# kkty/kmer-sets-compression

Hardware: AMD Instinct MI355X
Metric: Mk-mers/s processed in kmerset-multiple-compress; bytes/k-mer after SPSS (higher is better)
Workload: dtype u32

## Files before the change

kmer-sets-compression_amd/csrc/ksh_decode.hip:

```cpp
#include "ksh_internal.h"
#include "ksh_kmer.h"

#include <algorithm>
#include <cstdlib>
#include <string>
#include <vector>

namespace ksh {

constexpr int kDecThreads = 1024;
constexpr int kMaxLdsBuckets = 16384;
constexpr int kSortLdsBytes = 63488;
constexpr int kMaxSubBits = 11;
constexpr int kSortThreads = 1024;

__global__ __launch_bounds__(256) void k_str_bases(const uint32_t* __restrict__ lens, int64_t n,
                                                    int k, int64_t* __restrict__ bases) {
  const int64_t i = int64_t(blockIdx.x) * blockDim.x + threadIdx.x;
  if (i < n) bases[i] = int64_t(lens[i]) + k;
}

__global__ __launch_bounds__(256) void k_mark_ends(const int64_t* __restrict__ str_start,
                                                    int64_t n_strings,
                                                    unsigned long long* __restrict__ end_bits) {
// ... 46 lines not shown
    for (int j = 0; j < 32; j++) {
      const int64_t p = p0 + j;
      const bool valid = (p + k <= n_bases) && (((eb >> j) & no_end_mask) == 0);
      if (valid) {
        const uint64_t cn = (canonical_flag && rc < fw) ? rc : fw;
        const uint32_t bucket = uint32_t(cn >> key_bits);
        if (kScatter) {
          const uint32_t rel = atomicAdd(&lds_hist[bucket], 1u);
          keys[offsets[bucket] + rel] = KeyT(cn & key_mask);
        } else {
          atomicAdd(&lds_hist[bucket], 1u);
        }
      }
      const int q = j + k;
      const uint64_t nb = q < 32 ? (w0 >> (62 - 2 * q)) & 3 : (w1 >> (62 - 2 * (q - 32))) & 3;
      fw = ((fw << 2) & mask) | nb;
      rc = (rc >> 2) | ((3 - nb) << (2 * (k - 1)));
    }
  }
  if (!kScatter) {
    __syncthreads();
    for (int b = threadIdx.x; b < n_buckets; b += kDecThreads) my_row[b] = lds_hist[b];
  }
}

constexpr int kDecSgBits = 7;
constexpr int kDecL1Threads = 1024;
template <typename KeyT>
struct DecL1 {
  static constexpr int kPer = sizeof(KeyT) == 8 ? 4 : 8;
  static constexpr int kTile = kDecL1Threads * kPer;
};
constexpr int kDecL2Threads = 256;
constexpr int kDecL2Per = 8;
constexpr int kDecL2Tile = kDecL2Threads * kDecL2Per;

template <typename KeyT>
__global__ __launch_bounds__(kDecL1Threads) void k_decode_l1(
    const uint64_t* __restrict__ words, int64_t n_words, int64_t n_bases,
    const unsigned long long* __restrict__ end_bits, int64_t n_end_words, int k, int key_bits, int n_bucket_bits,
    int canonical_flag, int64_t words_per_group, const uint32_t* __restrict__ hist_matrix,
    const int64_t* __restrict__ offsets, KeyT* __restrict__ tmp_keys, uint16_t* __restrict__ tmp_b) {
  constexpr int kSg = 1 << kDecSgBits;
  constexpr int kDecL1Per = DecL1<KeyT>::kPer, kDecL1Tile = DecL1<KeyT>::kTile;
  constexpr int kParts = 32 / kDecL1Per;
  __shared__ KeyT s_key[kDecL1Tile];
  __shared__ uint16_t s_bkt[kDecL1Tile];
  __shared__ uint32_t s_cur[kSg], s_cnt[kSg], s_lbase[kSg + 1];
  const int tid = threadIdx.x;
  const int nb = 1 << n_bucket_bits, lo_bits = n_bucket_bits - kDecSgBits;
  const uint32_t* my_row = hist_matrix + int64_t(blockIdx.x) * nb;
  if (tid < kSg) {
    uint32_t at = uint32_t(offsets[int64_t(tid) << lo_bits]);
    for (int bi = 0; bi < (1 << lo_bits); bi++) at += my_row[(tid << lo_bits) + bi];
    s_cur[tid] = at;
    s_cnt[tid] = 0;
  }
  const int64_t w_begin = int64_t(blockIdx.x) * words_per_group;
  const int64_t w_end = min(w_begin + words_per_group, n_words);
  const uint64_t mask = kmer_mask(k);
  const uint64_t key_mask = (uint64_t(1) << key_bits) - 1;
  const uint64_t no_end_mask = (uint64_t(1) << (k - 1)) - 1;
  __syncthreads();
  for (int64_t w0i = w_begin; w0i < w_end; w0i += kDecL1Tile / 32) {
    const int64_t w = w0i + tid / kParts;
    const int j0 = (tid % kParts) * kDecL1Per;
    KeyT key[kDecL1Per];
    uint32_t bkt[kDecL1Per], rank[kDecL1Per];
// ... 36 lines not shown
      for (int d = 1; d < 64; d <<= 1) {
        const uint32_t o = __shfl_up(inc, d, 64);
        if (tid >= d) inc += o;
      }
      s_lbase[2 * tid] = inc - c0 - c1;
      s_lbase[2 * tid + 1] = inc - c1;
      if (tid == 63) s_lbase[kSg] = inc;
    }
    __syncthreads();
#pragma unroll
    for (int j = 0; j < kDecL1Per; j++) {
      if (bkt[j] == 0xFFFFFFFFu) continue;
      const uint32_t pos = s_lbase[bkt[j] >> lo_bits] + rank[j];
      s_key[pos] = key[j];
      s_bkt[pos] = uint16_t(bkt[j]);
    }
    __syncthreads();
    const int tile_n = int(s_lbase[kSg]);
    for (int i = tid; i < tile_n; i += kDecL1Threads) {
      const uint32_t sg = uint32_t(s_bkt[i]) >> lo_bits;
      const uint32_t dst = s_cur[sg] + (uint32_t(i) - s_lbase[sg]);
      tmp_keys[dst] = s_key[i];
      tmp_b[dst] = s_bkt[i];
    }
    __syncthreads();
    if (tid < kSg) {
      s_cur[tid] += s_cnt[tid];
      s_cnt[tid] = 0;
    }
    __syncthreads();
  }
}

template <typename KeyT>
__global__ __launch_bounds__(kDecL2Threads) void k_decode_l2(int64_t n, int n_bucket_bits,
                                                             const int64_t* __restrict__ offsets,
                                                             const KeyT* __restrict__ tmp_keys,
                                                             const uint16_t* __restrict__ tmp_b,
                                                             uint32_t* __restrict__ cursor, KeyT* __restrict__ keys) {
  constexpr int kBins = 2 * kDecL2Threads;
  __shared__ KeyT s_key[kDecL2Tile];
  __shared__ uint16_t s_bin[kDecL2Tile];
  __shared__ uint32_t s_cnt[kBins], s_lbase[kBins], s_gbase[kBins];
  __shared__ uint32_t s_wave[kDecL2Threads / 64];
  __shared__ uint32_t s_first;
  const int tid = threadIdx.x;
  const int lo_bits = n_bucket_bits - kDecSgBits;
  const int64_t p0 = int64_t(blockIdx.x) * kDecL2Tile;
  const int tile_n = int(min<int64_t>(kDecL2Tile, n - p0));
  s_cnt[2 * tid] = 0;
  s_cnt[2 * tid + 1] = 0;
  if (tid == 0) s_first = (uint32_t(tmp_b[p0]) >> lo_bits) << lo_bits;
  __syncthreads();
  const uint32_t base_b = s_first;
  const uint32_t n_bins = min<uint32_t>(uint32_t(kBins), (2u << lo_bits));
  KeyT mine[kDecL2Per];
  uint32_t bin[kDecL2Per], rank[kDecL2Per];
#pragma unroll
  for (int j = 0; j < kDecL2Per; j++) {
    const int i = tid + j * kDecL2Threads;
    bin[j] = 0xFFFFFFFFu;
    if (i >= tile_n) continue;
    mine[j] = tmp_keys[p0 + i];
    const uint32_t b = tmp_b[p0 + i];
    if (b - base_b < n_bins) {
      bin[j] = b - base_b;
      rank[j] = atomicAdd(&s_cnt[bin[j]], 1u);
    } else {
      keys[uint32_t(offsets[b]) + atomicAdd(&cursor[b], 1u)] = mine[j];
    }
  }
  __syncthreads();
  {
    const uint32_t c0 = s_cnt[2 * tid], c1 = s_cnt[2 * tid + 1];
    uint32_t inc = c0 + c1;
    const int lane = tid & 63, wv = tid >> 6;
#pragma unroll
    for (int d = 1; d < 64; d <<= 1) {
      const uint32_t o = __shfl_up(inc, d, 64);
      if (lane >= d) inc += o;
    }
    if (lane == 63) s_wave[wv] = inc;
    __syncthreads();
    uint32_t before = inc - (c0 + c1);
    for (int w = 0; w < wv; w++) before += s_wave[w];
    s_lbase[2 * tid] = before;
    s_lbase[2 * tid + 1] = before + c0;
    s_gbase[2 * tid] = c0 ? uint32_t(offsets[base_b + 2 * tid]) + atomicAdd(&cursor[base_b + 2 * tid], c0) : 0u;
    s_gbase[2 * tid + 1] = c1 ? uint32_t(offsets[base_b + 2 * tid + 1]) + atomicAdd(&cursor[base_b + 2 * tid + 1], c1) : 0u;
  }
  __syncthreads();
#pragma unroll
  for (int j = 0; j < kDecL2Per; j++) {
    if (bin[j] == 0xFFFFFFFFu) continue;
    const uint32_t pos = s_lbase[bin[j]] + rank[j];
    s_key[pos] = mine[j];
    s_bin[pos] = uint16_t(bin[j]);
  }
  __syncthreads();
  const uint32_t staged = s_lbase[kBins - 1] + s_cnt[kBins - 1];
  for (uint32_t i = tid; i < staged; i += kDecL2Threads) {
    const uint32_t b = s_bin[i];
    keys[s_gbase[b] + (i - s_lbase[b])] = s_key[i];
  }
}

constexpr int kColTeams = 16;
__global__ __launch_bounds__(64 * kColTeams) void k_hist_columns(uint32_t* __restrict__ hist_matrix,
                                                                  int64_t n_groups, int n_buckets,
                                                                  int64_t* __restrict__ totals,
                                                                  unsigned long long* __restrict__ max_total) {
  __shared__ uint32_t team_total[kColTeams][64];
  const int lane = threadIdx.x & 63, team = threadIdx.x >> 6;
  const int b = blockIdx.x * 64 + lane;
  const int64_t per_team = (n_groups + kColTeams - 1) / kColTeams;
  const int64_t g0 = min(int64_t(team) * per_team, n_groups), g1 = min(g0 + per_team, n_groups);
  uint32_t run = 0;
  if (b < n_buckets)
    for (int64_t g = g0; g < g1; g++) run += hist_matrix[g * n_buckets + b];
  team_total[team][lane] = run;
  __syncthreads();
  if (b >= n_buckets) return;
  uint32_t before = 0, all = 0;
#pragma unroll
  for (int t2 = 0; t2 < kColTeams; t2++) {
    const uint32_t v = team_total[t2][lane];
// ... 1 lines not shown
    all += v;
  }
  run = before;
  for (int64_t g = g0; g < g1; g++) {
    uint32_t* cell = hist_matrix + g * n_buckets + b;
    const uint32_t c = *cell;
    *cell = run;
    run += c;
  }
  if (team == 0) {
    totals[b] = all;
    unsigned long long m = all;
    if (int(blockIdx.x + 1) * 64 <= n_buckets) {
#pragma unroll
      for (int d = 32; d >= 1; d >>= 1) {
        const unsigned long long o = __shfl_xor(m, d, 64);
        m = o > m ? o : m;
      }
      if (lane == 0 && max_total) atomicMax(max_total, m);
    } else if (max_total) {
      atomicMax(max_total, m);
    }
  }
}

struct SortLds {
  uint32_t sub_cnt[(1 << kMaxSubBits) + 1];
  int wave_cnt[kSortThreads / 64];
  int wave_below[kSortThreads / 64];
  int overflow;
  int kept;
};

template <typename KeyT>
__device__ void block_sort_into_lds(const KeyT* __restrict__ src, int cnt, int eff_bits,
                                    KeyT* __restrict__ lds, SortLds* __restrict__ sh) {
  int bits = 0;
  while ((4 << bits) < cnt && bits < kMaxSubBits) bits++;
  if (bits > eff_bits) bits = eff_bits;
  const int n_sub = 1 << bits;
  const int shift = eff_bits - bits;
  for (int i = threadIdx.x; i <= n_sub; i += kSortThreads) sh->sub_cnt[i] = 0;
  if (threadIdx.x == 0) sh->overflow = 0;
  constexpr int kSortRegs = 8;
  const bool in_regs = cnt <= kSortRegs * kSortThreads;
  KeyT held[kSortRegs];
  if (in_regs) {
#pragma unroll
    for (int u = 0; u < kSortRegs; u++) {
      const int i = int(threadIdx.x) + u * kSortThreads;
      if (i < cnt) held[u] = src[i];
    }
  }
  __syncthreads();
  if (in_regs) {
#pragma unroll
    for (int u = 0; u < kSortRegs; u++)
      if (int(threadIdx.x) + u * kSortThreads < cnt)
        atomicAdd(&sh->sub_cnt[uint32_t(uint64_t(held[u]) >> shift) & uint32_t(n_sub - 1)], 1u);
  } else {
    for (int i = threadIdx.x; i < cnt; i += kSortThreads)
      atomicAdd(&sh->sub_cnt[uint32_t(uint64_t(src[i]) >> shift) & uint32_t(n_sub - 1)], 1u);
  }
  __syncthreads();
  {
    const int per = (n_sub + kSortThreads - 1) / kSortThreads;
    const int c0 = min(int(threadIdx.x) * per, n_sub), c1 = min(c0 + per, n_sub);
// ... 4 lines not shown
#pragma unroll
    for (int d = 1; d < 64; d <<= 1) {
      const int o = __shfl_up(inc, d, 64);
      if (lane >= d) inc += o;
    }
    if (lane == 63) sh->wave_cnt[wave] = inc;
    __syncthreads();
    int run = inc - mine;
    for (int w = 0; w < wave; w++) run += sh->wave_cnt[w];
    for (int i = c0; i < c1; i++) {
      const int c = int(sh->sub_cnt[i]);
      sh->sub_cnt[i] = uint32_t(run);
      run += c;
    }
  }
  __syncthreads();
  if (in_regs) {
#pragma unroll
    for (int u = 0; u < kSortRegs; u++)
      if (int(threadIdx.x) + u * kSortThreads < cnt) {
        const uint32_t pos = atomicAdd(&sh->sub_cnt[uint32_t(uint64_t(held[u]) >> shift) & uint32_t(n_sub - 1)], 1u);
        lds[pos] = held[u];
      }
  } else {
    for (int i = threadIdx.x; i < cnt; i += kSortThreads) {
      const KeyT key = src[i];
      const uint32_t pos = atomicAdd(&sh->sub_cnt[uint32_t(uint64_t(key) >> shift) & uint32_t(n_sub - 1)], 1u);
      lds[pos] = key;
    }
  }
  __syncthreads();
  for (int b2 = threadIdx.x; b2 < n_sub; b2 += kSortThreads) {
    const int s0 = b2 ? int(sh->sub_cnt[b2 - 1]) : 0, s1 = int(sh->sub_cnt[b2]);
    if (s1 - s0 > 64) {
      sh->overflow = 1;
    } else {
      for (int i = s0 + 1; i < s1; i++) {
        const KeyT x = lds[i];
        int j = i - 1;
        while (j >= s0 && lds[j] > x) {
          lds[j + 1] = lds[j];
          j--;
        }
        lds[j + 1] = x;
      }
    }
  }
  __syncthreads();
  if (sh->overflow == 0) return;
  int padded = 1;
  while (padded < cnt) padded <<= 1;
  const int half = padded >> 1;
  for (int size = 2; size <= padded; size <<= 1) {
    const int hs = size >> 1;
    for (int p = threadIdx.x; p < half; p += kSortThreads) {
      const int block = p / hs, o = p - block * hs;
      const int i = block * size + o, j = block * size + size - 1 - o;
      if (j < cnt) {
        const KeyT x = lds[i], y = lds[j];
        if (x > y) {
          lds[i] = y;
          lds[j] = x;
        }
      }
    }
    __syncthreads();
    for (int stride = size >> 2; stride > 0; stride >>= 1) {
      for (int p = threadIdx.x; p < half; p += kSortThreads) {
// ... 39 lines not shown
#pragma unroll
  for (int d = 32; d >= 1; d >>= 1) inc_below += __shfl_xor(inc_below, d, 64);
  __syncthreads();
  if (lane == 63) sh->wave_cnt[wave] = inc;
  if (lane == 0) sh->wave_below[wave] = inc_below;
  __syncthreads();
  int at = inc - mine;
  for (int w = 0; w < wave; w++) at += sh->wave_cnt[w];
  int total = 0;
#pragma unroll
  for (int w = 0; w < kSortThreads / 64; w++) total += sh->wave_cnt[w];
  if (threadIdx.x == 0 && below)
    for (int w = 0; w < kSortThreads / 64; w++) *below += sh->wave_below[w];
  if (total == cnt) {
    for (int i = threadIdx.x; i < cnt; i += kSortThreads) dst[i] = lds[i];
    __syncthreads();
    return total;
  }
  for (int i = c0; i < c1; i++) {
    if (i == 0 || lds[i] != lds[i - 1]) {
      bool keep = true;
      if (cutoff > 1) {
        int run = 1;
        while (run < cutoff && i + run < cnt && lds[i + run] == lds[i]) run++;
        keep = run >= cutoff;
      }
      if (keep) dst[at++] = lds[i];
    }
  }
  __syncthreads();
  return total;
}

template <typename KeyT>
__global__ __launch_bounds__(kSortThreads, 8) void k_bucket_sort(const int64_t* __restrict__ offsets,
                                                      KeyT* __restrict__ keys,
                                                      KeyT* __restrict__ scratch,
                                                      int64_t* __restrict__ uniq, int key_bits,
                                                      int cutoff, int64_t* __restrict__ below) {
  extern __shared__ unsigned char lds_raw[];
  __shared__ SortLds sh;
  __shared__ uint32_t part_end[(1 << kMaxSubBits) + 1];
  KeyT* lds = reinterpret_cast<KeyT*>(lds_raw);
  constexpr int kCap = kSortLdsBytes / int(sizeof(KeyT));
  const int64_t b = blockIdx.x;
  const int64_t lo = offsets[b], hi = offsets[b + 1];
  const int64_t cnt64 = hi - lo;
  if (cnt64 == 0) {
    if (threadIdx.x == 0) {
      uniq[b] = 0;
      if (below) below[b] = 0;
    }
    return;
  }
  KeyT* g = keys + lo;
  int64_t n_below = 0;
  if (cnt64 <= kCap) {
    block_sort_into_lds(g, int(cnt64), key_bits, lds, &sh);
    const int kept = block_unique_write(lds, int(cnt64), g, &sh, cutoff, &n_below);
    if (threadIdx.x == 0) {
      uniq[b] = kept;
      if (below) below[b] = n_below;
    }
    return;
  }
  KeyT* tmp = scratch + lo;
  int bits = 1;
  while ((cnt64 >> bits) > kCap / 4 && bits < kMaxSubBits) bits++;
  if (bits > key_bits) bits = key_bits;
  const int n_part = 1 << bits;
  const int shift = key_bits - bits;
  for (int i = threadIdx.x; i <= n_part; i += kSortThreads) part_end[i] = 0;
  __syncthreads();
  for (int64_t i = threadIdx.x; i < cnt64; i += kSortThreads)
    atomicAdd(&part_end[uint32_t(uint64_t(g[i]) >> shift) & uint32_t(n_part - 1)], 1u);
  __syncthreads();
  if (threadIdx.x == 0) {
    uint32_t run = 0;
    for (int i = 0; i < n_part; i++) {
      const uint32_t c = part_end[i];
      part_end[i] = run;
      run += c;
    }
  }
  __syncthreads();
  for (int64_t i = threadIdx.x; i < cnt64; i += kSortThreads) {
    const KeyT key = g[i];
    const uint32_t pos = atomicAdd(&part_end[uint32_t(uint64_t(key) >> shift) & uint32_t(n_part - 1)], 1u);
    tmp[pos] = key;
  }
  __syncthreads();
  int64_t out = 0;
  for (int p = 0; p < n_part; p++) {
    const int64_t s0 = p ? int64_t(part_end[p - 1]) : 0, s1 = int64_t(part_end[p]);
    const int64_t pc = s1 - s0;
    if (pc == 0) continue;
    if (pc <= kCap) {
      block_sort_into_lds(tmp + s0, int(pc), shift, lds, &sh);
      out += block_unique_write(lds, int(pc), g + out, &sh, cutoff, &n_below);
    } else {
      KeyT* buf = tmp + s0;
      int64_t padded = 1;
      while (padded < pc) padded <<= 1;
      const int64_t half = padded >> 1;
      for (int64_t size = 2; size <= padded; size <<= 1) {
        const int64_t hs = size >> 1;
        for (int64_t q = threadIdx.x; q < half; q += kSortThreads) {
          const int64_t block = q / hs, o = q - block * hs;
          const int64_t i = block * size + o, j = block * size + size - 1 - o;
          if (j < pc) {
            const KeyT x = buf[i], y = buf[j];
            if (x > y) {
              buf[i] = y;
              buf[j] = x;
            }
          }
        }
        __syncthreads();
        for (int64_t stride = size >> 2; stride > 0; stride >>= 1) {
          for (int64_t q = threadIdx.x; q < half; q += kSortThreads) {
            const int64_t i = 2 * stride * (q / stride) + (q % stride), j = i + stride;
            if (j < pc) {
              const KeyT x = buf[i], y = buf[j];
              if (x > y) {
                buf[i] = y;
                buf[j] = x;
              }
            }
          }
          __syncthreads();
        }
// ... 180 lines not shown
  ctx->dec_words = n_words;
  ctx->dec_groups = groups;
  ctx->dec_src = s->d_words;
  return KSH_OK;
}

template <typename KeyT>
int scatter_sort(ksh_ctx* ctx, const ksh_spss_view* s, const DecodeState& st, int k, int nbits_w, int kbw,
                 int canonical_flag, const int64_t* offsets, KeyT* keys, int cutoff, bool want_below,
                 int64_t** new_off, int64_t** below) {
  const int64_t nb = int64_t(1) << nbits_w;
  int64_t n_words, n_end_words, groups, wpg;
  decode_geometry(s, &n_words, &n_end_words, &groups, &wpg);
  static const bool direct = [] {
    const char* e = getenv("KSH_DECODE_SCATTER");
    return e && std::string(e) == "direct";
  }();
  static const int64_t two_level_min = [] {
    const char* e = getenv("KSH_DECODE_L2_MIN");
    return e ? std::max<int64_t>(1024, atoll(e)) : int64_t(1) << 20;
  }();
  if (!direct && ctx->dec_kmers >= two_level_min && nbits_w > kDecSgBits && nbits_w <= 15 &&
      ctx->dec_kmers < int64_t(0xFFFFFFF0)) {
    void* tmp = nullptr;
    const size_t tk = (size_t(ctx->dec_kmers) * sizeof(KeyT) + 255) & ~size_t(255);
    KSH_TRY(pool_alloc(ctx, tk + size_t(ctx->dec_kmers) * 2 + size_t(nb) * 4 + 256, &tmp));
    KeyT* tmp_keys = static_cast<KeyT*>(tmp);
    uint16_t* tmp_b = reinterpret_cast<uint16_t*>(static_cast<char*>(tmp) + tk);
    uint32_t* cursor = reinterpret_cast<uint32_t*>(static_cast<char*>(tmp) + tk + ((size_t(ctx->dec_kmers) * 2 + 255) & ~size_t(255)));
    KSH_HIP(hipMemsetAsync(cursor, 0, size_t(nb) * 4, ctx->stream));
    hipLaunchKernelGGL((k_decode_l1<KeyT>), dim3(unsigned(groups)), dim3(kDecL1Threads), 0, ctx->stream, s->d_words,
                       n_words, s->n_bases, st.end_bits, n_end_words, k, kbw, nbits_w,
                       canonical_flag, wpg, st.hist, offsets, tmp_keys, tmp_b);
    hipLaunchKernelGGL((k_decode_l2<KeyT>), dim3(unsigned((ctx->dec_kmers + kDecL2Tile - 1) / kDecL2Tile)),
                       dim3(kDecL2Threads), 0, ctx->stream, ctx->dec_kmers, nbits_w, offsets, tmp_keys, tmp_b,
                       cursor, keys);
    pool_free(ctx, tmp);
  } else {
    hipLaunchKernelGGL((k_decode<KeyT, true>), dim3(unsigned(groups)), dim3(kDecThreads),
                       size_t(nb) * 4, ctx->stream, s->d_words, n_words, s->n_bases, st.end_bits,
                       n_end_words, k, kbw, int(nb), canonical_flag, wpg, st.hist, offsets,
                       keys);
  }
  KeyT* scratch = nullptr;
  {
    const int64_t max_bucket = ctx->dec_max_bucket;
    if (max_bucket > int64_t(kSortLdsBytes / sizeof(KeyT))) {
      void* ptr = nullptr;
      KSH_TRY(pool_alloc(ctx, size_t(ctx->dec_kmers) * sizeof(KeyT), &ptr));
      scratch = static_cast<KeyT*>(ptr);
    }
  }
  arena_reset(ctx);
  KSH_TRY(arena_reserve(ctx, 2 * a256(size_t(nb + 1) * 8) + (1u << 16)));
  *new_off = static_cast<int64_t*>(arena_alloc(ctx, size_t(nb + 1) * 8));
  *below = static_cast<int64_t*>(arena_alloc(ctx, size_t(nb + 1) * 8));
  if (!*new_off || !*below) return fail(KSH_INTERNAL, "scratch arena too small");
  {
    const uint32_t bit = 8u << (sizeof(KeyT) == 2 ? 0 : sizeof(KeyT) == 4 ? 1 : 2);
    if (!(ctx->lds_opt_in & bit)) {
      KSH_HIP(hipFuncSetAttribute(reinterpret_cast<const void*>(k_bucket_sort<KeyT>),
                                  hipFuncAttributeMaxDynamicSharedMemorySize, kSortLdsBytes));
      ctx->lds_opt_in |= bit;
    }
  }
  hipLaunchKernelGGL((k_bucket_sort<KeyT>), dim3(unsigned(nb)), dim3(kSortThreads), kSortLdsBytes, ctx->stream,
                     offsets, keys, scratch, st.totals, kbw, cutoff, want_below ? *below : nullptr);
  if (scratch) pool_free(ctx, scratch);
  KSH_HIP(hipGetLastError());
  return KSH_OK;
}

template <typename KeyT, typename CT>
int decode_write_wide(ksh_ctx* ctx, const ksh_geom* g, const ksh_spss_view* s, int canonical_flag,
                      int64_t* d_offsets, void* d_keys, int64_t* n_keys, int cutoff, int64_t* n_below) {
  const int64_t nb = n_buckets(g), nbc = int64_t(1) << kCoarseBits;
  const int sub_bits = g->n_bucket_bits - kCoarseBits, cbits = 2 * g->k - kCoarseBits;
  int64_t n_words, n_end_words, groups, wpg;
  decode_geometry(s, &n_words, &n_end_words, &groups, &wpg);
  DecodeState st;
  decode_carve(ctx, groups, nbc, n_end_words, s->n_strings, &st);
  KeyT* keys = static_cast<KeyT*>(d_keys);
  constexpr bool in_place = sizeof(CT) == sizeof(KeyT);
  CT* comp = reinterpret_cast<CT*>(d_keys);
  if (!in_place) {
    void* ptr = nullptr;
    KSH_TRY(pool_alloc(ctx, size_t(ctx->dec_kmers) * sizeof(CT), &ptr));
    comp = static_cast<CT*>(ptr);
  }
  int64_t *new_off = nullptr, *below = nullptr;
  KSH_TRY(scatter_sort<CT>(ctx, s, st, g->k, kCoarseBits, cbits, canonical_flag, st.coarse, comp, cutoff,
                           n_below != nullptr, &new_off, &below));
  KSH_TRY(scan_exclusive_i64(ctx, st.totals, new_off, nbc, new_off + nbc));
  if (n_below) KSH_TRY(scan_exclusive_i64(ctx, below, below, nbc, below + nbc));
  hipLaunchKernelGGL((k_fine_offsets<CT>), dim3(unsigned(nb / 256 + 1)), dim3(256), 0, ctx->stream, st.coarse,
                     new_off, comp, sub_bits, key_bits(g), nb, d_offsets);
  KSH_HIP(hipMemcpyAsync(ctx->h_pinned, new_off + nbc, 8, hipMemcpyDeviceToHost, ctx->stream));
  if (n_below)
    KSH_HIP(hipMemcpyAsync(ctx->h_pinned + 1, below + nbc, 8, hipMemcpyDeviceToHost, ctx->stream));
  KSH_HIP(hipStreamSynchronize(ctx->stream));
// ... 139 lines not shown
```

kmer-sets-compression_amd/csrc/ksh_encode.hip:

```cpp
#include "ksh_internal.h"
#include "ksh_dsu.h"
#include "ksh_kmer.h"

#include <algorithm>
#include <cstddef>
#include <cstdlib>
#include <string>

namespace ksh {

#ifndef KSH_RULER_SHIFT
#define KSH_RULER_SHIFT 5
#endif
constexpr int kRulerShift = KSH_RULER_SHIFT;
constexpr uint32_t kRulerEvery = 1u << kRulerShift;

constexpr uint32_t kNone = 0xFFFFFFFFu;
constexpr uint32_t kMulti = 0xFFFFFFFEu;

#ifndef KSH_JUMP_HOPS
#define KSH_JUMP_HOPS 4
#endif
constexpr int kJumpHops = KSH_JUMP_HOPS;

// ... 204 lines not shown
                                                      RcRecord<KeyT>* __restrict__ rec) {
  extern __shared__ uint32_t lds_hist[];
  const int nb = 1 << nbits;
  const uint32_t* my_row = hist_matrix + int64_t(blockIdx.x) * nb;
  for (int b = threadIdx.x; b < nb; b += blockDim.x) lds_hist[b] = uint32_t(goff[b]) + my_row[b];
  const int64_t t_begin = int64_t(blockIdx.x) * per_row;
  const int64_t t_end = min(t_begin + per_row, set.n);
  __syncthreads();
  if (t_begin >= t_end) return;
  const int64_t b_first = set.bucket_of(t_begin), b_last = set.bucket_of(t_end - 1);
  const int k = set.k, low_bits = 2 * set.k - 2 - nbits;
  const uint64_t low_mask = (uint64_t(1) << low_bits) - 1;
  for (int64_t t = t_begin + threadIdx.x; t < t_end; t += blockDim.x) {
    const uint64_t key = uint64_t(set.keys[t]);
    const uint32_t grp = uint32_t(revcomp(key, k) >> low_bits) & uint32_t(nb - 1);
    if (int(grp >> (nbits - round_bits)) != round) continue;
    int64_t lo = b_first, hi = b_last;
    while (lo < hi) {
      const int64_t mid = (lo + hi + 1) >> 1;
      if (set.off[mid] <= t) lo = mid; else hi = mid - 1;
    }
    const uint64_t rx = revcomp((uint64_t(lo) << set.key_bits) | key, k);
    const uint32_t dst = atomicAdd(&lds_hist[grp], 1u);
    RcRecord<KeyT> r;
    r.key = KeyT(((rx >> (2 * k - 2)) << low_bits) | (rx & low_mask));
    r.t = uint32_t(t);
    rec[dst] = r;
  }
}

constexpr int kSgBits = 7;
constexpr int kL1Threads = 1024;
constexpr int kL2Threads = 256;
constexpr int kL2Per = 8;
constexpr int kL2Tile = kL2Threads * kL2Per;

template <typename KeyT, int kPer>
__global__ __launch_bounds__(kL1Threads) void k_rc_scatter_l1(DevSet<KeyT> set, int nbits, int64_t per_row,
                                                               const uint32_t* __restrict__ hist_matrix,
                                                               const int64_t* __restrict__ goff,
                                                               RcRecord<KeyT>* __restrict__ tmp_rec,
                                                               uint16_t* __restrict__ tmp_g) {
  constexpr int kTile = kL1Threads * kPer;
  constexpr int kSg = 1 << kSgBits;
  __shared__ RcRecord<KeyT> s_rec[kTile];
  __shared__ uint16_t s_g[kTile];
  __shared__ uint32_t s_cur[kSg], s_cnt[kSg], s_lbase[kSg + 1];
  constexpr int kOffCap = 1024;
  __shared__ int64_t s_off[kOffCap];
  const int tid = threadIdx.x;
  const int nb = 1 << nbits, lo_bits = nbits - kSgBits;
  const uint32_t* my_row = hist_matrix + int64_t(blockIdx.x) * nb;
  if (tid < kSg) {
    uint32_t at = uint32_t(goff[int64_t(tid) << lo_bits]);
    for (int gi = 0; gi < (1 << lo_bits); gi++) at += my_row[(tid << lo_bits) + gi];
    s_cur[tid] = at;
    s_cnt[tid] = 0;
  }
  const int64_t t_begin = int64_t(blockIdx.x) * per_row;
  const int64_t t_end = min(t_begin + per_row, set.n);
  __syncthreads();
  if (t_begin >= t_end) return;
  const int64_t b_first = set.bucket_of(t_begin), b_last = set.bucket_of(t_end - 1);
  const int k = set.k, low_bits = 2 * set.k - 2 - nbits;
  const uint64_t low_mask = (uint64_t(1) << low_bits) - 1;
  const int n_span = int(min<int64_t>(b_last - b_first + 1, kOffCap + 1));
  const bool off_staged = n_span <= kOffCap;
  if (off_staged)
// ... 36 lines not shown
      uint32_t inc = c0 + c1;
#pragma unroll
      for (int d = 1; d < 64; d <<= 1) {
        const uint32_t o = __shfl_up(inc, d, 64);
        if (tid >= d) inc += o;
      }
      s_lbase[2 * tid] = inc - c0 - c1;
      s_lbase[2 * tid + 1] = inc - c1;
    }
    __syncthreads();
#pragma unroll
    for (int j = 0; j < kPer; j++) {
      if (grp[j] == 0xFFFFFFFFu) continue;
      const uint32_t pos = s_lbase[grp[j] >> lo_bits] + rank[j];
      s_rec[pos] = mine[j];
      s_g[pos] = uint16_t(grp[j]);
    }
    __syncthreads();
    for (int i = tid; i < tile_n; i += kL1Threads) {
      const uint32_t sg = uint32_t(s_g[i]) >> lo_bits;
      const uint32_t dst = s_cur[sg] + (uint32_t(i) - s_lbase[sg]);
      tmp_rec[dst] = s_rec[i];
      tmp_g[dst] = s_g[i];
    }
    __syncthreads();
    if (tid < kSg) {
      s_cur[tid] += s_cnt[tid];
      s_cnt[tid] = 0;
    }
    __syncthreads();
  }
}

template <typename KeyT>
__global__ __launch_bounds__(kL2Threads) void k_rc_scatter_l2(int64_t n, int nbits, const int64_t* __restrict__ goff,
                                                               const RcRecord<KeyT>* __restrict__ tmp_rec,
                                                               const uint16_t* __restrict__ tmp_g,
                                                               uint32_t* __restrict__ cursor,
                                                               RcRecord<KeyT>* __restrict__ rec) {
  constexpr int kBins = 512;
  __shared__ RcRecord<KeyT> s_rec[kL2Tile];
  __shared__ uint16_t s_bin[kL2Tile];
  __shared__ uint32_t s_cnt[kBins], s_lbase[kBins], s_gbase[kBins];
  __shared__ uint32_t s_first;
  const int tid = threadIdx.x;
  const int lo_bits = nbits - kSgBits;
  const int64_t p0 = int64_t(blockIdx.x) * kL2Tile;
  const int tile_n = int(min<int64_t>(kL2Tile, n - p0));
  for (int b = tid; b < kBins; b += kL2Threads) s_cnt[b] = 0;
  if (tid == 0) s_first = (uint32_t(tmp_g[p0]) >> lo_bits) << lo_bits;
  __syncthreads();
  const uint32_t base_g = s_first;
  const uint32_t n_bins = min<uint32_t>(uint32_t(kBins), (2u << lo_bits));
  RcRecord<KeyT> mine[kL2Per];
  uint32_t bin[kL2Per], rank[kL2Per];
#pragma unroll
  for (int j = 0; j < kL2Per; j++) {
    const int i = tid + j * kL2Threads;
    bin[j] = 0xFFFFFFFFu;
    if (i >= tile_n) continue;
    mine[j] = tmp_rec[p0 + i];
    const uint32_t g = tmp_g[p0 + i];
    if (g - base_g < n_bins) {
      bin[j] = g - base_g;
      rank[j] = atomicAdd(&s_cnt[bin[j]], 1u);
    } else {
      rec[uint32_t(goff[g]) + atomicAdd(&cursor[g], 1u)] = mine[j];
    }
  }
  __syncthreads();
  {
    static_assert(kBins == 2 * kL2Threads, "two bins per thread");
    __shared__ uint32_t s_wave[kL2Threads / 64];
    const uint32_t c0 = s_cnt[2 * tid], c1 = s_cnt[2 * tid + 1];
    uint32_t inc = c0 + c1;
    const int lane = tid & 63, wv = tid >> 6;
#pragma unroll
    for (int d = 1; d < 64; d <<= 1) {
      const uint32_t o = __shfl_up(inc, d, 64);
      if (lane >= d) inc += o;
    }
    if (lane == 63) s_wave[wv] = inc;
    __syncthreads();
    uint32_t before = inc - (c0 + c1);
    for (int w = 0; w < wv; w++) before += s_wave[w];
    s_lbase[2 * tid] = before;
    s_lbase[2 * tid + 1] = before + c0;
    s_gbase[2 * tid] = c0 ? uint32_t(goff[base_g + 2 * tid]) + atomicAdd(&cursor[base_g + 2 * tid], c0) : 0u;
    s_gbase[2 * tid + 1] = c1 ? uint32_t(goff[base_g + 2 * tid + 1]) + atomicAdd(&cursor[base_g + 2 * tid + 1], c1) : 0u;
  }
  __syncthreads();
#pragma unroll
  for (int j = 0; j < kL2Per; j++) {
    if (bin[j] == 0xFFFFFFFFu) continue;
    const uint32_t pos = s_lbase[bin[j]] + rank[j];
    s_rec[pos] = mine[j];
    s_bin[pos] = uint16_t(bin[j]);
  }
  __syncthreads();
  uint32_t staged = 0;
  for (int b = 0; b < kBins; b++) staged += s_cnt[b];
  for (uint32_t i = tid; i < staged; i += kL2Threads) {
    const uint32_t b = s_bin[i];
    rec[s_gbase[b] + (i - s_lbase[b])] = s_rec[i];
  }
}

template <typename KeyT>
__device__ int64_t lower_bound_kmer(const DevSet<KeyT>& set, uint64_t value) {
  const int64_t b = int64_t(value >> set.key_bits);
  if (b >= set.n_buckets) return set.n;
  const KeyT key = KeyT(value & set.key_mask());
  int64_t lo, hi;
  set.probe_range(b, key, &lo, &hi);
  while (lo < hi) {
    const int64_t mid = (lo + hi) >> 1;
    if (set.keys[mid] < key) lo = mid + 1; else hi = mid;
  }
  return lo;
}

__device__ __forceinline__ void mark_hit(uint32_t* slot, uint32_t v) {
  if (atomicCAS(slot, kNone, v) != kNone) *reinterpret_cast<volatile uint32_t*>(slot) = kMulti;
}

constexpr int kRcSegs = 16;

template <typename KeyT>
__global__ __launch_bounds__(256) void k_rc_bounds(DevSet<KeyT> set, int nbits, int64_t* __restrict__ pb,
                                                    int64_t* __restrict__ pb0) {
  const int64_t i = int64_t(blockIdx.x) * blockDim.x + threadIdx.x;
  const int64_t n_pb = int64_t(2 * kRcSegs) << nbits;
  if (i < n_pb) {
    const uint64_t grp = uint64_t(i) >> 5, seg = (uint64_t(i) >> 1) & 15, which = uint64_t(i) & 1;
// ... 2706 lines not shown
          KSH_HIP(hipFuncSetAttribute(reinterpret_cast<const void*>(k_adj_rc<KeyT, 64>),
                                      hipFuncAttributeMaxDynamicSharedMemorySize, bytes));
          KSH_HIP(hipFuncSetAttribute(reinterpret_cast<const void*>(k_adj_rc1<KeyT, 1024>),
                                      hipFuncAttributeMaxDynamicSharedMemorySize, kRc1LdsBytes));
          KSH_HIP(hipFuncSetAttribute(reinterpret_cast<const void*>(k_adj_rc1<KeyT, 512>),
                                      hipFuncAttributeMaxDynamicSharedMemorySize, kRc1LdsBytes));
          KSH_HIP(hipFuncSetAttribute(reinterpret_cast<const void*>(k_adj_rc1<KeyT, 256>),
                                      hipFuncAttributeMaxDynamicSharedMemorySize, kRc1LdsBytes));
          KSH_HIP(hipFuncSetAttribute(reinterpret_cast<const void*>(k_adj_rc1<KeyT, 64>),
                                      hipFuncAttributeMaxDynamicSharedMemorySize, kRc1LdsBytes));
          KSH_HIP(hipFuncSetAttribute(reinterpret_cast<const void*>(k_rc_hist<KeyT>),
                                      hipFuncAttributeMaxDynamicSharedMemorySize, int(size_t(4) << 15)));
          ctx->lds_opt_in |= bit;
        }
      }
      KSH_BOUND(hist_lds <= (size_t(4) << 15) && ng <= 65536);
      hipLaunchKernelGGL((k_rc_hist<KeyT>), dim3(unsigned(rows)), dim3(1024), hist_lds, st,
                         static_cast<const KeyT*>(sv->d_keys), n, g->k, key_bits(g), gbits, per_row, hist);
      hipLaunchKernelGGL(k_rc_columns, dim3(unsigned((ng + 63) / 64)), dim3(64 * kColTeams), 0, st, hist, rows, int(ng),
                         totals);
      KSH_TRY(scan_exclusive_i64(ctx, totals, goff, ng, goff + ng));
      p->routes |= KSH_ROUTE_PROBE_STAGED | (two_level ? KSH_ROUTE_SCATTER_TWO_LEVEL : 0);
      if (two_level) {
        RcRecord<KeyT>* tmp_rec = sizeof(RcRecord<KeyT>) == 8 ? rec + n : reinterpret_cast<RcRecord<KeyT>*>(p->nbr);
        uint16_t* tmp_g = reinterpret_cast<uint16_t*>(p->head);
        KSH_BOUND(sizeof(RcRecord<KeyT>) == 8 ? size_t(2 * n) * sizeof(RcRecord<KeyT>) <= al(size_t(2 * n) * 8)
                                    : reinterpret_cast<char*>(p->link) == reinterpret_cast<char*>(p->nbr) + al(size_t(2 * n) * 4) &&
                                          size_t(n) * sizeof(RcRecord<KeyT>) <= 2 * al(size_t(2 * n) * 4));
        KSH_BOUND(gbits - kSgBits <= 8);
        uint32_t* cursor = rc_cursor;
        constexpr int kPer = sizeof(RcRecord<KeyT>) == 8 ? 4 : 2;
        hipLaunchKernelGGL((k_rc_scatter_l1<KeyT, kPer>), dim3(unsigned(rows)), dim3(kL1Threads), 0, st, set, gbits,
                           per_row, hist, goff, tmp_rec, tmp_g);
        hipLaunchKernelGGL((k_rc_scatter_l2<KeyT>), dim3(unsigned((n + kL2Tile - 1) / kL2Tile)), dim3(kL2Threads), 0,
                           st, n, gbits, goff, tmp_rec, tmp_g, cursor, rec);
      } else {
        hipLaunchKernelGGL((k_rc_scatter<KeyT>), dim3(unsigned(rows)), dim3(1024), hist_lds, st, set, gbits, 0, 0,
                           per_row, hist, goff, rec);
      }
      const int64_t per_group = n / ng;
      const int cap = int(std::min<int64_t>((kRcWindowBytes - 4 * kRcSegs) / int64_t(sizeof(KeyT) + 6),
                                            std::max<int64_t>(1024, extra ? per_group * 23 / 20 + 256 : per_group * 5 / 4 + 256))) & ~7;
      const size_t rc_lds = size_t(cap) * (sizeof(KeyT) + 4) + size_t(cap + 2 * kRcSegs) * 2;
      KSH_BOUND(cap >= 8 && cap % 8 == 0 && cap + 2 * kRcSegs < 65536);
      KSH_BOUND(rc_lds + 2048 <= size_t(kRcWindowBytes) + 2048 && rc_lds <= size_t(kRcWindowBytes));
      int64_t* pb = static_cast<int64_t*>(arena_alloc(ctx, size_t(ng) * 2 * kRcSegs * 8));
      int64_t* pb0 = extra ? static_cast<int64_t*>(arena_alloc(ctx, size_t(ng) * 2 * 8)) : nullptr;
      if (!pb || (extra && !pb0)) return fail(KSH_INTERNAL, "scratch arena too small");
      hipLaunchKernelGGL((k_rc_bounds<KeyT>), dim3(nblk(ng * 2 * kRcSegs + (extra ? ng * 2 : 0))), dim3(256), 0, st, set,
                         gbits, pb, pb0);
      p->routes |= per_group > 4096 ? KSH_ROUTE_RC_1024 : per_group > 1024 ? KSH_ROUTE_RC_512
                   : per_group > 256 ? KSH_ROUTE_RC_256 : KSH_ROUTE_RC_64;
      static const int rc1_mode = [] {
        const char* e = getenv("KSH_RC1");
        return !e ? 1 : (std::string(e) == "marks" ? 2 : (std::string(e) == "batched" ? 0 : 1));
      }();
      const bool rc1_marks = rc1_mode == 2;
      const int rc1_cap = rc1_marks ? 0 : int(std::min<int64_t>(Rc1Cfg<KeyT>::kCap, (per_group * 4 / 3 + 263) & ~int64_t(7)));
      const int pass1_cap = rc1_marks ? -1 : rc1_cap;
      const bool with_rc = rc1_mode != 0;
      int rc1_sbits = 6;
      while ((1 << rc1_sbits) < kRc1SlicesMax && (2 << rc1_sbits) <= rc1_cap + 1) rc1_sbits++;
      const size_t rc1_lds = (size_t(4) << rc1_sbits) + size_t(rc1_cap) * Rc1Cfg<KeyT>::kEntryBytes;
      KSH_BOUND(rc1_lds <= size_t(kRc1LdsBytes) && rc1_cap % 8 == 0 && rc1_cap < (2 << rc1_sbits) - 1);
      if (!rc1_marks) p->routes |= KSH_ROUTE_RC1_STREAMED;
      const int rc1_batched = rc1_mode == 0 ? 1 : 0;
#define KSH_LAUNCH_RC(T)                                                                                              \
  do {                                                                                                                \
// ... 583 lines not shown
```

kmer-sets-compression_amd/csrc/ksh_internal.h:

```cpp
#ifndef KSH_INTERNAL_H_
#define KSH_INTERNAL_H_

#include <hip/hip_runtime.h>

#include <cstdarg>
#include <cstdint>
#include <cstdio>
#include <functional>
#include <map>
#include <mutex>
#include <string>
#include <unordered_map>
#include <vector>

#include "kmersets_hip.h"

namespace ksh {

void set_error(const char* fmt, ...);
int fail(int code, const char* fmt, ...);

#define KSH_HIP(expr)                                                                   \
  do {                                                                                  \
    hipError_t err__ = (expr);                                                          \
    if (err__ != hipSuccess)                                                            \
      return ::ksh::fail(KSH_INTERNAL, "%s failed: %s (%s:%d)", #expr,                  \
                         hipGetErrorString(err__), __FILE__, __LINE__);                 \
  } while (0)

#define KSH_BY_KEY(key_bytes, FN, ...)                                   \
  ((key_bytes) == 2 ? FN<uint16_t>(__VA_ARGS__)                          \
                    : (key_bytes) == 4 ? FN<uint32_t>(__VA_ARGS__) : FN<uint64_t>(__VA_ARGS__))

#define KSH_TRY(expr)              \
  do {                             \
    int rc__ = (expr);             \
    if (rc__ != KSH_OK) return rc__; \
  } while (0)

constexpr int kNumTimers = 8;

}

struct ksh_ctx {
  int device = 0;
  hipStream_t stream = nullptr;
  bool own_stream = false;

  char* arena = nullptr;
  size_t arena_bytes = 0;
  size_t arena_used = 0;

  int64_t* h_pinned = nullptr;
// ... 120 lines not shown
```

Before: 27730.

## Double L2 scatter tile for small keys and add register bitonic sort of sub-bins

```diff
diff --git a/kmer-sets-compression_amd/csrc/ksh_decode.hip b/kmer-sets-compression_amd/csrc/ksh_decode.hip
--- a/kmer-sets-compression_amd/csrc/ksh_decode.hip
+++ b/kmer-sets-compression_amd/csrc/ksh_decode.hip
@@ -102,8 +102,6 @@
   static constexpr int kTile = kDecL1Threads * kPer;
 };
 constexpr int kDecL2Threads = 256;
-constexpr int kDecL2Per = 8;
-constexpr int kDecL2Tile = kDecL2Threads * kDecL2Per;
 
 template <typename KeyT>
 __global__ __launch_bounds__(kDecL1Threads) void k_decode_l1(
@@ -206,32 +204,33 @@
   }
 }
 
-template <typename KeyT>
+template <typename KeyT, int kPer>
 __global__ __launch_bounds__(kDecL2Threads) void k_decode_l2(int64_t n, int n_bucket_bits,
                                                              const int64_t* __restrict__ offsets,
                                                              const KeyT* __restrict__ tmp_keys,
                                                              const uint16_t* __restrict__ tmp_b,
                                                              uint32_t* __restrict__ cursor, KeyT* __restrict__ keys) {
+  constexpr int kTile = kDecL2Threads * kPer;
   constexpr int kBins = 2 * kDecL2Threads;
-  __shared__ KeyT s_key[kDecL2Tile];
-  __shared__ uint16_t s_bin[kDecL2Tile];
+  __shared__ KeyT s_key[kTile];
+  __shared__ uint16_t s_bin[kTile];
   __shared__ uint32_t s_cnt[kBins], s_lbase[kBins], s_gbase[kBins];
   __shared__ uint32_t s_wave[kDecL2Threads / 64];
   __shared__ uint32_t s_first;
   const int tid = threadIdx.x;
   const int lo_bits = n_bucket_bits - kDecSgBits;
-  const int64_t p0 = int64_t(blockIdx.x) * kDecL2Tile;
-  const int tile_n = int(min<int64_t>(kDecL2Tile, n - p0));
+  const int64_t p0 = int64_t(blockIdx.x) * kTile;
+  const int tile_n = int(min<int64_t>(kTile, n - p0));
   s_cnt[2 * tid] = 0;
   s_cnt[2 * tid + 1] = 0;
   if (tid == 0) s_first = (uint32_t(tmp_b[p0]) >> lo_bits) << lo_bits;
   __syncthreads();
   const uint32_t base_b = s_first;
   const uint32_t n_bins = min<uint32_t>(uint32_t(kBins), (2u << lo_bits));
-  KeyT mine[kDecL2Per];
-  uint32_t bin[kDecL2Per], rank[kDecL2Per];
-#pragma unroll
-  for (int j = 0; j < kDecL2Per; j++) {
+  KeyT mine[kPer];
+  uint32_t bin[kPer], rank[kPer];
+#pragma unroll
+  for (int j = 0; j < kPer; j++) {
     const int i = tid + j * kDecL2Threads;
     bin[j] = 0xFFFFFFFFu;
     if (i >= tile_n) continue;
@@ -265,7 +264,7 @@
   }
   __syncthreads();
 #pragma unroll
-  for (int j = 0; j < kDecL2Per; j++) {
+  for (int j = 0; j < kPer; j++) {
     if (bin[j] == 0xFFFFFFFFu) continue;
     const uint32_t pos = s_lbase[bin[j]] + rank[j];
     s_key[pos] = mine[j];
@@ -333,7 +332,36 @@
   int kept;
 };
 
-template <typename KeyT>
+template <typename KeyT, int M>
+__device__ __forceinline__ void reg_sort(KeyT (&v)[M]) {
+#pragma unroll
+  for (int size = 2; size <= M; size <<= 1)
+#pragma unroll
+    for (int stride = size >> 1; stride > 0; stride >>= 1)
+#pragma unroll
+      for (int i = 0; i < M; i++) {
+        const int j = i ^ stride;
+        if (j > i) {
+          const KeyT lo = v[i] < v[j] ? v[i] : v[j], hi = v[i] < v[j] ? v[j] : v[i];
+          const bool up = (i & size) == 0;
+          v[i] = up ? lo : hi;
+          v[j] = up ? hi : lo;
+        }
+      }
+}
+
+template <typename KeyT, int M>
+__device__ __forceinline__ void sort_sub_bin_regs(KeyT* __restrict__ lds, int s0, int n) {
+  KeyT v[M];
+#pragma unroll
+  for (int u = 0; u < M; u++) v[u] = u < n ? lds[s0 + u] : KeyT(~KeyT(0));
+  reg_sort<KeyT, M>(v);
+#pragma unroll
+  for (int u = 0; u < M; u++)
+    if (u < n) lds[s0 + u] = v[u];
+}
+
+template <typename KeyT, bool kRegSort>
 __device__ void block_sort_into_lds(const KeyT* __restrict__ src, int cnt, int eff_bits,
                                     KeyT* __restrict__ lds, SortLds* __restrict__ sh) {
   int bits = 0;
@@ -404,8 +432,13 @@
   __syncthreads();
   for (int b2 = threadIdx.x; b2 < n_sub; b2 += kSortThreads) {
     const int s0 = b2 ? int(sh->sub_cnt[b2 - 1]) : 0, s1 = int(sh->sub_cnt[b2]);
-    if (s1 - s0 > 64) {
+    const int n = s1 - s0;
+    if (n > 64) {
       sh->overflow = 1;
+    } else if (kRegSort && !__any(n > 16)) {
+      if (__any(n > 8)) sort_sub_bin_regs<KeyT, 16>(lds, s0, n);
+      else if (__any(n > 4)) sort_sub_bin_regs<KeyT, 8>(lds, s0, n);
+      else if (__any(n > 1)) sort_sub_bin_regs<KeyT, 4>(lds, s0, n);
     } else {
       for (int i = s0 + 1; i < s1; i++) {
         const KeyT x = lds[i];
@@ -511,7 +544,7 @@
   return total;
 }
 
-template <typename KeyT>
+template <typename KeyT, bool kRegSort>
 __global__ __launch_bounds__(kSortThreads, 8) void k_bucket_sort(const int64_t* __restrict__ offsets,
                                                       KeyT* __restrict__ keys,
                                                       KeyT* __restrict__ scratch,
@@ -535,7 +568,7 @@
   KeyT* g = keys + lo;
   int64_t n_below = 0;
   if (cnt64 <= kCap) {
-    block_sort_into_lds(g, int(cnt64), key_bits, lds, &sh);
+    block_sort_into_lds<KeyT, kRegSort>(g, int(cnt64), key_bits, lds, &sh);
     const int kept = block_unique_write(lds, int(cnt64), g, &sh, cutoff, &n_below);
     if (threadIdx.x == 0) {
       uniq[b] = kept;
@@ -575,7 +608,7 @@
     const int64_t pc = s1 - s0;
     if (pc == 0) continue;
     if (pc <= kCap) {
-      block_sort_into_lds(tmp + s0, int(pc), shift, lds, &sh);
+      block_sort_into_lds<KeyT, kRegSort>(tmp + s0, int(pc), shift, lds, &sh);
       out += block_unique_write(lds, int(pc), g + out, &sh, cutoff, &n_below);
     } else {
       KeyT* buf = tmp + s0;
@@ -822,9 +855,14 @@
     hipLaunchKernelGGL((k_decode_l1<KeyT>), dim3(unsigned(groups)), dim3(kDecL1Threads), 0, ctx->stream, s->d_words,
                        n_words, s->n_bases, st.end_bits, n_end_words, k, kbw, nbits_w,
                        canonical_flag, wpg, st.hist, offsets, tmp_keys, tmp_b);
-    hipLaunchKernelGGL((k_decode_l2<KeyT>), dim3(unsigned((ctx->dec_kmers + kDecL2Tile - 1) / kDecL2Tile)),
-                       dim3(kDecL2Threads), 0, ctx->stream, ctx->dec_kmers, nbits_w, offsets, tmp_keys, tmp_b,
-                       cursor, keys);
+    if (sizeof(KeyT) <= 4 && scatter_l2_tile() != 2048)
+      hipLaunchKernelGGL((k_decode_l2<KeyT, 16>), dim3(unsigned((ctx->dec_kmers + 4095) / 4096)),
+                         dim3(kDecL2Threads), 0, ctx->stream, ctx->dec_kmers, nbits_w, offsets, tmp_keys, tmp_b,
+                         cursor, keys);
+    else
+      hipLaunchKernelGGL((k_decode_l2<KeyT, 8>), dim3(unsigned((ctx->dec_kmers + 2047) / 2048)),
+                         dim3(kDecL2Threads), 0, ctx->stream, ctx->dec_kmers, nbits_w, offsets, tmp_keys, tmp_b,
+                         cursor, keys);
     pool_free(ctx, tmp);
   } else {
     hipLaunchKernelGGL((k_decode<KeyT, true>), dim3(unsigned(groups)), dim3(kDecThreads),
@@ -846,16 +884,27 @@
   *new_off = static_cast<int64_t*>(arena_alloc(ctx, size_t(nb + 1) * 8));
   *below = static_cast<int64_t*>(arena_alloc(ctx, size_t(nb + 1) * 8));
   if (!*new_off || !*below) return fail(KSH_INTERNAL, "scratch arena too small");
+  constexpr bool kRegs = sizeof(KeyT) < 8;
   {
     const uint32_t bit = 8u << (sizeof(KeyT) == 2 ? 0 : sizeof(KeyT) == 4 ? 1 : 2);
     if (!(ctx->lds_opt_in & bit)) {
-      KSH_HIP(hipFuncSetAttribute(reinterpret_cast<const void*>(k_bucket_sort<KeyT>),
+      KSH_HIP(hipFuncSetAttribute(reinterpret_cast<const void*>(k_bucket_sort<KeyT, kRegs>),
+                                  hipFuncAttributeMaxDynamicSharedMemorySize, kSortLdsBytes));
+      KSH_HIP(hipFuncSetAttribute(reinterpret_cast<const void*>(k_bucket_sort<KeyT, false>),
                                   hipFuncAttributeMaxDynamicSharedMemorySize, kSortLdsBytes));
       ctx->lds_opt_in |= bit;
     }
   }
-  hipLaunchKernelGGL((k_bucket_sort<KeyT>), dim3(unsigned(nb)), dim3(kSortThreads), kSortLdsBytes, ctx->stream,
-                     offsets, keys, scratch, st.totals, kbw, cutoff, want_below ? *below : nullptr);
+  static const bool insertion = [] {
+    const char* e = getenv("KSH_DECODE_SORT");
+    return e && std::string(e) == "insertion";
+  }();
+  if (!insertion)
+    hipLaunchKernelGGL((k_bucket_sort<KeyT, kRegs>), dim3(unsigned(nb)), dim3(kSortThreads), kSortLdsBytes,
+                       ctx->stream, offsets, keys, scratch, st.totals, kbw, cutoff, want_below ? *below : nullptr);
+  else
+    hipLaunchKernelGGL((k_bucket_sort<KeyT, false>), dim3(unsigned(nb)), dim3(kSortThreads), kSortLdsBytes,
+                       ctx->stream, offsets, keys, scratch, st.totals, kbw, cutoff, want_below ? *below : nullptr);
   if (scratch) pool_free(ctx, scratch);
   KSH_HIP(hipGetLastError());
   return KSH_OK;
diff --git a/kmer-sets-compression_amd/csrc/ksh_encode.hip b/kmer-sets-compression_amd/csrc/ksh_encode.hip
--- a/kmer-sets-compression_amd/csrc/ksh_encode.hip
+++ b/kmer-sets-compression_amd/csrc/ksh_encode.hip
@@ -260,8 +260,6 @@
 constexpr int kSgBits = 7;
 constexpr int kL1Threads = 1024;
 constexpr int kL2Threads = 256;
-constexpr int kL2Per = 8;
-constexpr int kL2Tile = kL2Threads * kL2Per;
 
 template <typename KeyT, int kPer>
 __global__ __launch_bounds__(kL1Threads) void k_rc_scatter_l1(DevSet<KeyT> set, int nbits, int64_t per_row,
@@ -364,30 +362,31 @@
   }
 }
 
-template <typename KeyT>
+template <typename KeyT, int kPer>
 __global__ __launch_bounds__(kL2Threads) void k_rc_scatter_l2(int64_t n, int nbits, const int64_t* __restrict__ goff,
                                                                const RcRecord<KeyT>* __restrict__ tmp_rec,
                                                                const uint16_t* __restrict__ tmp_g,
                                                                uint32_t* __restrict__ cursor,
                                                                RcRecord<KeyT>* __restrict__ rec) {
+  constexpr int kTile = kL2Threads * kPer;
   constexpr int kBins = 512;
-  __shared__ RcRecord<KeyT> s_rec[kL2Tile];
-  __shared__ uint16_t s_bin[kL2Tile];
+  __shared__ RcRecord<KeyT> s_rec[kTile];
+  __shared__ uint16_t s_bin[kTile];
   __shared__ uint32_t s_cnt[kBins], s_lbase[kBins], s_gbase[kBins];
   __shared__ uint32_t s_first;
   const int tid = threadIdx.x;
   const int lo_bits = nbits - kSgBits;
-  const int64_t p0 = int64_t(blockIdx.x) * kL2Tile;
-  const int tile_n = int(min<int64_t>(kL2Tile, n - p0));
+  const int64_t p0 = int64_t(blockIdx.x) * kTile;
+  const int tile_n = int(min<int64_t>(kTile, n - p0));
   for (int b = tid; b < kBins; b += kL2Threads) s_cnt[b] = 0;
   if (tid == 0) s_first = (uint32_t(tmp_g[p0]) >> lo_bits) << lo_bits;
   __syncthreads();
   const uint32_t base_g = s_first;
   const uint32_t n_bins = min<uint32_t>(uint32_t(kBins), (2u << lo_bits));
-  RcRecord<KeyT> mine[kL2Per];
-  uint32_t bin[kL2Per], rank[kL2Per];
-#pragma unroll
-  for (int j = 0; j < kL2Per; j++) {
+  RcRecord<KeyT> mine[kPer];
+  uint32_t bin[kPer], rank[kPer];
+#pragma unroll
+  for (int j = 0; j < kPer; j++) {
     const int i = tid + j * kL2Threads;
     bin[j] = 0xFFFFFFFFu;
     if (i >= tile_n) continue;
@@ -423,15 +422,14 @@
   }
   __syncthreads();
 #pragma unroll
-  for (int j = 0; j < kL2Per; j++) {
+  for (int j = 0; j < kPer; j++) {
     if (bin[j] == 0xFFFFFFFFu) continue;
     const uint32_t pos = s_lbase[bin[j]] + rank[j];
     s_rec[pos] = mine[j];
     s_bin[pos] = uint16_t(bin[j]);
   }
   __syncthreads();
-  uint32_t staged = 0;
-  for (int b = 0; b < kBins; b++) staged += s_cnt[b];
+  const uint32_t staged = s_lbase[kBins - 1] + s_cnt[kBins - 1];
   for (uint32_t i = tid; i < staged; i += kL2Threads) {
     const uint32_t b = s_bin[i];
     rec[s_gbase[b] + (i - s_lbase[b])] = s_rec[i];
@@ -3204,8 +3202,12 @@
         constexpr int kPer = sizeof(RcRecord<KeyT>) == 8 ? 4 : 2;
         hipLaunchKernelGGL((k_rc_scatter_l1<KeyT, kPer>), dim3(unsigned(rows)), dim3(kL1Threads), 0, st, set, gbits,
                            per_row, hist, goff, tmp_rec, tmp_g);
-        hipLaunchKernelGGL((k_rc_scatter_l2<KeyT>), dim3(unsigned((n + kL2Tile - 1) / kL2Tile)), dim3(kL2Threads), 0,
-                           st, n, gbits, goff, tmp_rec, tmp_g, cursor, rec);
+        if (sizeof(RcRecord<KeyT>) == 8 && scatter_l2_tile() != 2048)
+          hipLaunchKernelGGL((k_rc_scatter_l2<KeyT, 16>), dim3(unsigned((n + 4095) / 4096)), dim3(kL2Threads), 0,
+                             st, n, gbits, goff, tmp_rec, tmp_g, cursor, rec);
+        else
+          hipLaunchKernelGGL((k_rc_scatter_l2<KeyT, 8>), dim3(unsigned((n + 2047) / 2048)), dim3(kL2Threads), 0,
+                             st, n, gbits, goff, tmp_rec, tmp_g, cursor, rec);
       } else {
         hipLaunchKernelGGL((k_rc_scatter<KeyT>), dim3(unsigned(rows)), dim3(1024), hist_lds, st, set, gbits, 0, 0,
                            per_row, hist, goff, rec);
diff --git a/kmer-sets-compression_amd/csrc/ksh_internal.h b/kmer-sets-compression_amd/csrc/ksh_internal.h
--- a/kmer-sets-compression_amd/csrc/ksh_internal.h
+++ b/kmer-sets-compression_amd/csrc/ksh_internal.h
@@ -6,6 +6,7 @@
 #include <cstdarg>
 #include <cstdint>
 #include <cstdio>
+#include <cstdlib>
 #include <functional>
 #include <map>
 #include <mutex>
@@ -19,6 +20,14 @@
 
 void set_error(const char* fmt, ...);
 int fail(int code, const char* fmt, ...);
+
+inline int scatter_l2_tile() {
+  static const int t = [] {
+    const char* e = std::getenv("KSH_SCATTER_L2_TILE");
+    return e ? std::atoi(e) : 0;
+  }();
+  return t;
+}
 
 #define KSH_HIP(expr)                                                                   \
   do {                                                                                  \
```

Result: no change. 27960, median of 6 (+0.8%).
